# LUMC/kPAL

Hardware: AMD Instinct MI355X
Metric: Gbases/s k-mer counted (k=12, 150bp synthetic) (higher is better)
Workload: dtype int64

## Files before the change

### kpal_amd/csrc/kpal_device.hpp

```cpp
#pragma once
#include <hip/hip_runtime.h>
#include <stdint.h>

namespace kpal {

__host__ __device__ inline uint64_t mix64(uint64_t x)
{
    uint64_t z = x + 0x9E3779B97F4A7C15ULL;
    z = (z ^ (z >> 30)) * 0xBF58476D1CE4E5B9ULL;
    z = (z ^ (z >> 27)) * 0x94D049BB133111EBULL;
    return z ^ (z >> 31);
}

__host__ __device__ inline uint64_t revcomp(uint64_t x, int k)
{
    uint64_t y = ~x;
#if defined(__HIP_DEVICE_COMPILE__)
    y = __brevll(y);
#else
    y = ((y >> 1) & 0x5555555555555555ULL) | ((y & 0x5555555555555555ULL) << 1);
    y = ((y >> 2) & 0x3333333333333333ULL) | ((y & 0x3333333333333333ULL) << 2);
    y = ((y >> 4) & 0x0F0F0F0F0F0F0F0FULL) | ((y & 0x0F0F0F0F0F0F0F0FULL) << 4);
    y = ((y >> 8) & 0x00FF00FF00FF00FFULL) | ((y & 0x00FF00FF00FF00FFULL) << 8);
    y = ((y >> 16) & 0x0000FFFF0000FFFFULL) | ((y & 0x0000FFFF0000FFFFULL) << 16);
    y = (y >> 32) | (y << 32);
#endif
    y = ((y >> 1) & 0x5555555555555555ULL) | ((y & 0x5555555555555555ULL) << 1);
    return y >> (64 - 2 * k);
}

__device__ __forceinline__ void classify4(uint32_t w, uint32_t &t, uint32_t &nz)
{
    t = ((w >> 1) ^ (w >> 2)) & 0x03030303u;
    const uint32_t expect = __builtin_amdgcn_perm(0u, 0x54474341u , t);
    const uint32_t x = (w & 0xDFDFDFDFu) ^ expect;
    nz = (((x & 0x7F7F7F7Fu) + 0x7F7F7F7Fu) | x) & 0x80808080u;
}

template <int SH>
__device__ __forceinline__ uint32_t shl_or(uint32_t a, uint32_t b)
{
    uint32_t r;
    asm("v_lshl_or_b32 %0, %1, %2, %3" : "=v"(r) : "v"(a), "n"(SH), "v"(b));
    return r;
}

__device__ __forceinline__ uint32_t codes_to_top_byte(uint32_t t)
{
    const uint32_t x = shl_or<10>(t, t);
    return shl_or<20>(x, x);
}

__device__ __forceinline__ uint32_t flags_to_top_byte(uint32_t m)
{
    const uint32_t x = shl_or<9>(m, m);
    return shl_or<18>(x, x);
}

__device__ __forceinline__ void encode4(uint32_t w, uint32_t &code8, uint32_t &bad4)
{
    uint32_t t, nz;
    classify4(w, t, nz);
    code8 = codes_to_top_byte(t) >> 24;
    bad4 = flags_to_top_byte(nz >> 7) >> 24;
}

struct Chunk {
    uint32_t codes;
    uint32_t bad;
};

__device__ __forceinline__ Chunk encode16(uint4 v)
{
    uint32_t t0, t1, t2, t3, z0, z1, z2, z3;
    classify4(v.x, t0, z0);
    classify4(v.y, t1, z1);
    classify4(v.z, t2, z2);
    classify4(v.w, t3, z3);
    Chunk r;
#if defined(KPAL_ENCODE_SHIFTS)
    const uint32_t c0 = codes_to_top_byte(t0), c1 = codes_to_top_byte(t1), c2 = codes_to_top_byte(t2), c3 = codes_to_top_byte(t3);
    const uint32_t c01 = __builtin_amdgcn_perm(c0, c1, 0x07030000u);
    const uint32_t c23 = __builtin_amdgcn_perm(c2, c3, 0x07030000u);
    const uint32_t f01 = flags_to_top_byte((z0 >> 3) | (z1 >> 7));
    const uint32_t f23 = flags_to_top_byte((z2 >> 3) | (z3 >> 7));
    r.codes = __builtin_amdgcn_perm(c01, c23, 0x07060302u);
    r.bad = __builtin_amdgcn_perm(f01, f23, 0x0c0c0703u);
#else
    constexpr uint32_t kDigits = 0x01041040u;
    const uint32_t d0 = __builtin_amdgcn_udot4(t0, kDigits, 0u, false), d1 = __builtin_amdgcn_udot4(t1, kDigits, 0u, false);
    const uint32_t d2 = __builtin_amdgcn_udot4(t2, kDigits, 0u, false), d3 = __builtin_amdgcn_udot4(t3, kDigits, 0u, false);
    r.codes = (d0 << 24) | ((d1 << 16) | ((d2 << 8) | d3));
    constexpr uint32_t kHigh = 0x10204080u, kLow = 0x01020408u;
    const uint32_t f01 = __builtin_amdgcn_udot4(z1, kLow, __builtin_amdgcn_udot4(z0, kHigh, 0u, false), false);
    const uint32_t f23 = __builtin_amdgcn_udot4(z3, kLow, __builtin_amdgcn_udot4(z2, kHigh, 0u, false), false);
    r.bad = (f01 << 1) | (f23 >> 7);
#endif
    return r;
}

struct Span {
    const uint4 *base;
    uint64_t lo;
    uint64_t hi;
    uint64_t emit_from;
    uint64_t nchunks;
};

__device__ __forceinline__ uint4 fetch_chunk(const Span &s, int64_t c)
{
    if (c < 0 || (uint64_t)c >= s.nchunks) return make_uint4(0u, 0u, 0u, 0u);
    return s.base[c];
}

__device__ __forceinline__ void range_fix(const Span &s, int64_t c, Chunk &r)
{
    if (c < 0 || (uint64_t)c >= s.nchunks) {
        r.codes = 0;
        r.bad = 0xFFFFu;
        return;
    }
    const uint64_t p0 = (uint64_t)c * 16;
    if (p0 < s.lo || p0 + 16 > s.hi) {
        const uint32_t a = s.lo > p0 ? (uint32_t)(s.lo - p0) : 0u;
        const uint32_t b = s.hi < p0 + 16 ? (uint32_t)(s.hi > p0 ? s.hi - p0 : 0) : 16u;
        const uint32_t in_range = (a < b) ? (((1u << (16 - a)) - 1u) & ~((1u << (16 - b)) - 1u)) : 0u;
        r.bad |= ~in_range & 0xFFFFu;
    }
}

__device__ __forceinline__ Chunk load_chunk(const Span &s, int64_t c)
{
    Chunk r = encode16(fetch_chunk(s, c));
    range_fix(s, c, r);
    return r;
}

template <int K>
__device__ __forceinline__ uint32_t emit_mask(uint32_t prev_bad, uint32_t cur_bad)
{
    uint32_t b = (prev_bad << 16) | cur_bad;
    uint32_t s = b;
    int have = 1;
#pragma unroll
    for (int step = 1; step < 32; step <<= 1) {
        if (have * 2 <= K) {
            s |= s >> have;
            have *= 2;
        }
    }
    if (have < K) s |= s >> (K - have);
    return ~s & 0xFFFFu;
}

__device__ __forceinline__ uint32_t emit_mask_rt(int k, uint32_t prev_bad, uint32_t cur_bad)
{
    uint32_t b = (prev_bad << 16) | cur_bad;
    uint32_t s = b;
    int have = 1;
    while (have * 2 <= k) {
        s |= s >> have;
        have *= 2;
    }
    if (have < k) s |= s >> (k - have);
    return ~s & 0xFFFFu;
}

__device__ __forceinline__ uint32_t emit_from_mask(const Span &s, int64_t c)
{
    const uint64_t p0 = (uint64_t)c * 16;
    if (s.emit_from <= p0) return 0xFFFFu;
    if (s.emit_from >= p0 + 16) return 0u;
    return (1u << (16 - (uint32_t)(s.emit_from - p0))) - 1u;
}

__device__ __forceinline__ uint32_t from_left_lane(uint32_t v, uint32_t lane0_value)
{
    return (uint32_t)__builtin_amdgcn_update_dpp((int)lane0_value, (int)v, 0x138 , 0xF, 0xF, false);
}

template <int K, bool EDGE>
__device__ __forceinline__ void wave_step(const Span &s, int64_t c, Chunk &carry, uint64_t &window,
                                          uint32_t &mask)
{
    Chunk cur;
    if constexpr (EDGE) cur = load_chunk(s, c);
    else cur = encode16(s.base[c]);
    const uint32_t pc = from_left_lane(cur.codes, carry.codes);
    const uint32_t pb = from_left_lane(cur.bad, carry.bad);
    carry.codes = __builtin_amdgcn_readlane(cur.codes, 63);
    carry.bad = __builtin_amdgcn_readlane(cur.bad, 63);
    window = ((uint64_t)pc << 32) | cur.codes;
    mask = emit_mask<K>(pb, cur.bad);
    if constexpr (EDGE) mask &= emit_from_mask(s, c);
}

template <int K>
__device__ __forceinline__ void encode_step(const Span &s, uint64_t step, const uint4 raw, Chunk &carry,
                                            uint64_t &window, uint32_t &mask, bool edge)
{
    const int lane = threadIdx.x & 63;
    const int64_t c = (int64_t)(step * 64 + lane);
    Chunk cur = encode16(raw);
    if (edge) range_fix(s, c, cur);
    const uint32_t pc = from_left_lane(cur.codes, carry.codes);
    const uint32_t pb = from_left_lane(cur.bad, carry.bad);
    carry.codes = __builtin_amdgcn_readlane(cur.codes, 63);
    carry.bad = __builtin_amdgcn_readlane(cur.bad, 63);
    window = ((uint64_t)pc << 32) | cur.codes;
    mask = emit_mask<K>(pb, cur.bad);
    if (edge) mask &= emit_from_mask(s, c);
}

__device__ __forceinline__ bool interior_steps(const Span &s, uint64_t step0, uint64_t step1)
{
    return step0 * 64 >= 1 && (step0 * 64 - 1) * 16 >= s.lo && step1 * 64 * 16 <= s.hi && s.emit_from <= step0 * 64 * 16;
}

template <int K>
__device__ __forceinline__ void encode_step(const Span &s, uint64_t step, const uint4 raw, Chunk &carry,
                                            uint64_t &window, uint32_t &mask)
{
    encode_step<K>(s, step, raw, carry, window, mask, !interior_steps(s, step, step + 1));
}

__device__ __forceinline__ bool interior_range(const Span &s, uint64_t c0, uint64_t c1)
{
    return c0 >= 1 && (c0 - 1) * 16 >= s.lo && c1 * 16 <= s.hi && s.emit_from <= c0 * 16;
}

template <int K>
__device__ __forceinline__ uint32_t kmer_at(uint64_t window, int j)
{
    constexpr uint64_t M = (K >= 16) ? 0xFFFFFFFFULL : ((1ULL << (2 * K)) - 1ULL);
    return (uint32_t)((window >> (2 * (15 - j))) & M);
}

template <int K>
__device__ __forceinline__ void part_step(const Span &s, uint64_t step, Chunk &carry, uint64_t &window, uint32_t &mask)
{
    const int lane = threadIdx.x & 63;
    if (interior_range(s, step * 64, step * 64 + 64)) wave_step<K, false>(s, (int64_t)(step * 64 + lane), carry, window, mask);
    else wave_step<K, true>(s, (int64_t)(step * 64 + lane), carry, window, mask);
}

__device__ __forceinline__ void lds_barrier()
{
    asm volatile("s_waitcnt lgkmcnt(0)\n\ts_barrier" ::: "memory");
}

}
```

### kpal_amd/csrc/quad_kernels.hpp

```cpp
#pragma once
#include <type_traits>

#include "kpal_device.hpp"
#include "quad2_index.hpp"

namespace kpal {

constexpr int kQuadSpillCap = 2048;
constexpr int kQuadRowWords = 32768;
constexpr int kQuadDummyWords = 4;

template <int K>
struct QuadCfg {
    static_assert(K >= 8 && K <= 16, "quads: k = 8..16");
    static constexpr bool kTwoLevel = K >= 13;
    static constexpr bool kStaged = K >= 12;
    static constexpr int kCoarseBits = kTwoLevel ? 2 * K - 22 : 0;
    static constexpr int kCoarse = 1 << kCoarseBits;
    static constexpr int kRep = kTwoLevel ? (kCoarse >= 256 ? 1 : 256 / kCoarse) : 1;
    static constexpr int kBucketBits = kTwoLevel ? 9 : (K == 12 ? 11 : 9);
    static constexpr int kHistBuckets = 1 << kBucketBits;
    static constexpr int kBuckets = kTwoLevel ? kCoarse * kRep : (1 << kBucketBits);
    static constexpr int kLowBits = kTwoLevel ? 13 : 2 * K - kBucketBits;
    static constexpr int kFormBins = 1 << kLowBits;
    static constexpr int kSlots = kQuadRowWords / kBuckets;
    static constexpr int kRecordBytes = kSlots * 4;
#if defined(KPAL_QUAD_ITEM4)
    static constexpr bool kItem3 = false;
#else
    static constexpr bool kItem3 = !kTwoLevel && K == 12;
#endif
    static constexpr int kItems = kItem3 ? (kSlots / 4) * 5 : kSlots;
#if defined(KPAL_QUAD_NO_PAIR)
    static constexpr bool kPairRows = false;
#else
    static constexpr bool kPairRows = !kTwoLevel && kRecordBytes == 64;
#endif
    static constexpr int kScrBits = (kLowBits - 6) < 4 ? (kLowBits - 6) : 4;
    static constexpr uint64_t kXMask = (1ull << (2 * K + 6)) - 1ull;
    static constexpr uint32_t kLowMask = (1u << kLowBits) - 1u;
    __host__ __device__ static constexpr uint32_t smask(uint32_t t)
    {
        return kScrBits > 0 ? (((t << (kBucketBits - kScrBits)) | t) & (uint32_t)((1 << kBucketBits) - 1)) : 0u;
    }
    __host__ __device__ static constexpr uint32_t smask1(uint32_t t) { return (kCoarseBits > 4 ? ((t << (kCoarseBits - 4)) ^ t) : t) & (uint32_t)(kCoarse - 1); }
};

static_assert(Quad2Index<13>::smask(11) == QuadCfg<13>::smask(11) && Quad2Index<16>::smask(5) == QuadCfg<16>::smask(5) &&
                  Quad2Index<13>::smask1(9) == QuadCfg<13>::smask1(9) && Quad2Index<14>::smask1(13) == QuadCfg<14>::smask1(13) &&
                  Quad2Index<15>::smask1(7) == QuadCfg<15>::smask1(7) && Quad2Index<16>::smask1(15) == QuadCfg<16>::smask1(15) &&
                  Quad2Index<15>::CB == QuadCfg<15>::kCoarseBits &&
                  ((Quad2Index<12>::smask1(13) << 9) | Quad2Index<12>::smask(13)) == QuadCfg<12>::smask(13) &&
                  ((Quad2Index<12>::smask1(6) << 9) | Quad2Index<12>::smask(6)) == QuadCfg<12>::smask(6),
              "quad2_index.hpp restates the scramble masks of QuadCfg");

template <int K>
__device__ __forceinline__ void quad_split(uint64_t x, uint32_t m4, uint32_t lane, uint32_t &row, uint32_t &item)
{
    using C = QuadCfg<K>;
    const uint32_t low = (uint32_t)x & C::kLowMask;
    const uint32_t hi6 = (uint32_t)(x >> (2 * K));
    if constexpr (C::kTwoLevel) {
        const uint32_t fine = ((uint32_t)x >> 13) & 511u;
        const uint32_t coarse = (uint32_t)(x >> 22) & (uint32_t)(C::kCoarse - 1);
        row = (coarse ^ C::smask1(low >> 9)) * C::kRep + (lane & (uint32_t)(C::kRep - 1));
        item = (hi6 << 26) | (fine << 17) | (low << 4) | m4;
    } else {
        const uint32_t b = ((uint32_t)x >> C::kLowBits) & (uint32_t)(C::kBuckets - 1);
        row = b ^ C::smask(low >> (C::kLowBits - C::kScrBits));
        item = (hi6 << (C::kLowBits + 4)) | (low << 4) | m4;
    }
}

template <int K, int LEVEL = 1>
__device__ __forceinline__ uint32_t quad_kmer(uint32_t row, uint32_t item, int i, uint32_t coarse = 0)
{
    using C = QuadCfg<K>;
    uint64_t x;
    if constexpr (LEVEL == 2) {
        const uint32_t low = (item >> 4) & 8191u, hi6 = item >> 17, t = low >> 9;
        x = ((uint64_t)hi6 << (2 * K)) | ((uint64_t)(coarse ^ C::smask1(t)) << 22) | ((uint64_t)(row ^ C::smask(t)) << 13) | low;
    } else if constexpr (C::kTwoLevel) {
        const uint32_t low = (item >> 4) & 8191u, fine = (item >> 17) & 511u, hi6 = item >> 26, t = low >> 9;
        x = ((uint64_t)hi6 << (2 * K)) | ((uint64_t)((row / C::kRep) ^ C::smask1(t)) << 22) | ((uint64_t)fine << 13) | low;
    } else {
        const uint32_t low = (item >> 4) & C::kLowMask;
        const uint32_t hi6 = item >> (C::kLowBits + 4);
        const uint32_t b = row ^ C::smask(low >> (C::kLowBits - C::kScrBits));
        x = ((uint64_t)hi6 << (2 * K)) | ((uint64_t)b << C::kLowBits) | low;
    }
    return (uint32_t)((x >> (6 - 2 * i)) & ((1ull << (2 * K)) - 1ull));
}

struct QuadPacked {
    uint32_t a, b, c;
};
__device__ __forceinline__ QuadPacked quad_pack3(const uint4 &v)
{
    QuadPacked r;
    r.a = v.x | (v.y << 23);
    r.b = (v.y >> 9) | (v.z << 14);
    r.c = (v.z >> 18) | (v.w << 5);
    return r;
}
__device__ __forceinline__ uint4 quad_unpack3(uint32_t a, uint32_t b, uint32_t c)
{
    uint4 v;
    v.x = a & 0x7FFFFFu;
    v.y = __builtin_amdgcn_alignbit(b, a, 23) & 0x7FFFFFu;
    v.z = __builtin_amdgcn_alignbit(c, b, 14) & 0x7FFFFFu;
    v.w = (c >> 5) & 0x7FFFFFu;
    return v;
}
constexpr int kQuadPackedRecordBytes = 192;

struct QuadSpill {
    uint32_t row, item;
};

struct QuadHot {
    unsigned long long key;
    uint32_t count, pad;
};
constexpr int kQuadHotEntries = 256;

struct TableSink {
    unsigned long long *table;
    unsigned long long *list;
    uint32_t *count;
    uint32_t cap;
    uint32_t *overflow;
};

struct TableOnly {
    unsigned long long *table;
};

__device__ __forceinline__ void sink_add(const TableOnly &sink, uint64_t index, unsigned long long n) { atomicAdd(&sink.table[index], n); }

struct TableSinkRef {
    const TableSink *p;
};

__device__ __forceinline__ void sink_add(const TableSink &sink, uint64_t index, unsigned long long n);
__device__ __forceinline__ void sink_add(const TableSinkRef &ref, uint64_t index, unsigned long long n) { sink_add(*ref.p, index, n); }

__device__ __forceinline__ void sink_add(const TableSink &sink, uint64_t index, unsigned long long n)
{
    if (sink.table) {
        atomicAdd(&sink.table[index], n);
    } else {
        const uint32_t at = atomicAdd(sink.count, 1u);
        if (at < sink.cap) sink.list[at] = ((unsigned long long)index << 32) | (n & 0xFFFFFFFFull);
        else *sink.overflow = 1u;
    }
}

__device__ __forceinline__ uint32_t quad_hot_hash(uint32_t row, uint32_t item)
{
    return ((item >> 4) * 0x9E3779B1u + row * 0x85EBCA6Bu) >> 24;
}

template <typename SINK>
__device__ __attribute__((noinline)) void quad_hot_age(const SINK table, QuadHot *hot)
{
    const QuadHot h = hot[threadIdx.x];
    if (h.key >> 63) {
        if (h.count == h.pad) {
            sink_add(table, (uint64_t)(h.key & 0x7FFFFFFFFFFFFFFFull), (unsigned long long)h.count);
            hot[threadIdx.x] = QuadHot{0ull, 0u, 0u};
        } else {
            hot[threadIdx.x].pad = h.count;
        }
    }
}

template <typename SINK>
__device__ __forceinline__ void quad_kmer_add(const SINK table, QuadHot *hot, uint64_t index, uint32_t n)
{
#if defined(KPAL_AB_DIRECT_NO_TABLE)
    return;
#endif
    const unsigned long long key = (1ull << 63) | (unsigned long long)index;
    const uint32_t h = ((uint32_t)index * 0x9E3779B1u + (uint32_t)(index >> 32)) >> 24;
    bool done = false;
#pragma unroll 1
    for (uint32_t pr = 0; pr < 4u && !done; ++pr) {
        const uint32_t slot = (h + pr) & (uint32_t)(kQuadHotEntries - 1);
        unsigned long long cur = hot[slot].key;
        if (cur == 0ull) {
            cur = atomicCAS(&hot[slot].key, 0ull, key);
            if (cur == 0ull) cur = key;
        }
        if (cur == key) {
            atomicAdd(&hot[slot].count, n);
            done = true;
        }
    }
    if (!done) sink_add(table, index, (unsigned long long)n);
}

template <int K, int LEVEL = 1, typename SINK = TableOnly, bool COUNTED = false, bool KMERS = false>
__device__ __forceinline__ void quad_items_direct_body(bool active, uint32_t row, uint32_t item, const SINK table, QuadHot *hot, uint32_t coarse = 0,
                                                       uint32_t cnt = 1u)
{
    const uint32_t mult = COUNTED ? cnt : 1u;
    const int lane = threadIdx.x & 63;
    auto kmer_add = [&](uint64_t index, uint32_t n) {
        if constexpr (KMERS) quad_kmer_add<SINK>(table, hot, index, n);
        else sink_add(table, index, (unsigned long long)n);
    };
    auto to_table = [&](uint32_t r, uint32_t it, uint32_t n) {
#pragma unroll
        for (int i = 0; i < 4; ++i)
            if ((it >> (3 - i)) & 1u) sink_add(table, quad_kmer<K, LEVEL>(r, it, i, coarse), (unsigned long long)n);
    };
    unsigned long long todo = __builtin_amdgcn_ballot_w64(active);
    for (int round = 0; round < 8 && todo; ++round) {
        const int src = __ffsll((long long)todo) - 1;
        const uint32_t hot_row = (uint32_t)__builtin_amdgcn_readlane(row, src);
        const uint32_t hot_item = (uint32_t)__builtin_amdgcn_readlane(item, src);
        const unsigned long long same = __builtin_amdgcn_ballot_w64(active && row == hot_row && item == hot_item) & todo;
        uint32_t n = (uint32_t)__popcll(same);
        if constexpr (COUNTED) {
            n = 0;
#pragma unroll
            for (uint32_t v = 1; v <= 4u; ++v) n += v * (uint32_t)__popcll(same & __builtin_amdgcn_ballot_w64(cnt == v));
        }
        const unsigned long long key = ((unsigned long long)hot_row << 32) | hot_item;
        const uint32_t slot = (quad_hot_hash(hot_row, hot_item) + (uint32_t)(lane & 3)) & (uint32_t)(kQuadHotEntries - 1);
        const unsigned long long seen = lane < 4 ? hot[slot].key : ~0ull;
        const unsigned long long hit = __builtin_amdgcn_ballot_w64(seen == key);
        if (hit) {
            if (lane == __ffsll((long long)hit) - 1) atomicAdd(&hot[slot].count, n);
        } else {
            const unsigned long long free_slots = __builtin_amdgcn_ballot_w64(seen == 0ull);
            bool placed = false;
            if (n >= 2u && free_slots) {
                const int who = __ffsll((long long)free_slots) - 1;
                const unsigned long long old = lane == who ? atomicCAS(&hot[slot].key, 0ull, key) : 1ull;
                placed = __builtin_amdgcn_ballot_w64(lane == who && (old == 0ull || old == key)) != 0ull;
                if (placed && lane == who) atomicAdd(&hot[slot].count, n);
            }
            if constexpr (KMERS) {
                if (!placed && lane < 4 && ((hot_item >> (3 - lane)) & 1u)) kmer_add(quad_kmer<K, LEVEL>(hot_row, hot_item, lane, coarse), n);
            } else {
                if (!placed && lane == src) to_table(hot_row, hot_item, n);
            }
        }
        todo &= ~same;
    }
    if ((todo >> lane) & 1ull) {
        const unsigned long long key = ((unsigned long long)row << 32) | item;
        const uint32_t h = quad_hot_hash(row, item);
        bool done = false;
#pragma unroll
        for (int pr = 0; pr < 4 && !done; ++pr) {
            const uint32_t slot = (h + (uint32_t)pr) & (uint32_t)(kQuadHotEntries - 1);
            if (hot[slot].key == key) {
                atomicAdd(&hot[slot].count, mult);
                done = true;
            }
        }
        if (!done) to_table(row, item, mult);
    }
}

template <int K, int LEVEL = 1, typename SINK = TableOnly, bool KM = false>
__device__ __attribute__((noinline)) void quad_items_direct(bool active, uint32_t row, uint32_t item, const SINK table, QuadHot *hot, uint32_t coarse = 0)
{
    quad_items_direct_body<K, LEVEL, SINK, false, KM>(active, row, item, table, hot, coarse);
}

template <int K, typename SINK>
__device__ __attribute__((noinline)) void quad_items_direct_counted(uint32_t cnt, uint32_t row, uint32_t item, const SINK table, QuadHot *hot)
{
    quad_items_direct_body<K, 1, SINK, true, true>(cnt != 0u, row, item, table, hot, 0u, cnt);
}

template <int K, bool DIRECT = false, int LEVEL = 1, int N = 4, typename SINK = TableOnly, bool KM = false>
__device__ __forceinline__ uint32_t quad_place(uint32_t *rows, uint32_t *pos, QuadSpill *spill, uint32_t *spill_n, uint32_t cap,
                                               const uint32_t (&row)[N], const uint32_t (&item)[N], const SINK &table,
                                               QuadHot *hot, uint32_t coarse = 0)
{
    using C = typename std::conditional<LEVEL == 2, QuadCfg<11>, QuadCfg<K>>::type;
    constexpr uint32_t RB = (uint32_t)C::kSlots * 4u;
    constexpr bool ITEM3 = LEVEL == 1 && C::kItem3;
    uint32_t riders = 0;
    uint32_t off[N];
#pragma unroll
    for (int q = 0; q < N; ++q) off[q] = atomicAdd(&pos[row[q]], (item[q] & 15u) ? 4u : 0u);
    uint32_t over = 0;
#pragma unroll
    for (int q = 0; q < N; ++q) {
        const bool counted = (item[q] & 15u) != 0u;
        if constexpr (ITEM3) {
            const bool normal = off[q] < RB;
            const bool rider = !normal && off[q] < RB + RB / 4;
            if (counted && normal) atomicOr(reinterpret_cast<uint32_t *>(reinterpret_cast<char *>(rows) + row[q] * RB + off[q]), item[q]);
            riders |= (counted && rider) ? (1u << q) : 0u;
            over |= (counted && !normal && !rider) ? (1u << q) : 0u;
        } else {
            const bool fits = off[q] < RB;
            const uint32_t at = row[q] * RB + off[q];
            *reinterpret_cast<uint32_t *>(reinterpret_cast<char *>(rows) + ((counted && fits) ? at : (uint32_t)kQuadRowWords * 4u)) = item[q];
            over |= (counted && !fits) ? (1u << q) : 0u;
        }
    }
#if defined(KPAL_AB_SCATTER_NO_RIDER)
    riders = 0;
#endif
#if defined(KPAL_AB_SCATTER_NO_SPILL)
    over = 0;
#endif
    if constexpr (ITEM3) {
        if (__any(riders != 0u)) {
#pragma unroll
            for (int q = 0; q < N; ++q)
                if ((riders >> q) & 1u) {
                    uint32_t *p = reinterpret_cast<uint32_t *>(reinterpret_cast<char *>(rows) + row[q] * RB + (off[q] - RB) * 4u);
#if defined(KPAL_AB_RIDER_OR)
                    atomicOr(p, item[q] << 24);
                    atomicOr(p + 1, (item[q] << 16) & 0xFF000000u);
                    atomicOr(p + 2, (item[q] << 8) & 0xFF000000u);
#else
                    reinterpret_cast<unsigned char *>(p)[3] = (unsigned char)item[q];
                    reinterpret_cast<unsigned char *>(p)[7] = (unsigned char)(item[q] >> 8);
                    reinterpret_cast<unsigned char *>(p)[11] = (unsigned char)(item[q] >> 16);
#endif
                }
        }
    }
    if (__builtin_expect(__any(over != 0u), 0)) {
#if defined(KPAL_QUAD_NO_CARRY)
        constexpr bool direct = true;
#else
        constexpr bool direct = DIRECT;
#endif
#if defined(KPAL_AB_SPILL_LANE)
        if constexpr (!direct) {
            uint32_t at[N];
#pragma unroll
            for (int q = 0; q < N; ++q) at[q] = cap;
            if (over) {
#pragma unroll
                for (int q = 0; q < N; ++q)
                    if ((over >> q) & 1u) at[q] = atomicAdd(spill_n, 1u);
            }
            uint32_t unlisted = 0;
#pragma unroll
            for (int q = 0; q < N; ++q) {
                const bool ov = (over >> q) & 1u;
                if (ov && at[q] < cap) spill[at[q]] = QuadSpill{row[q], item[q]};
                unlisted |= (ov && at[q] >= cap) ? (1u << q) : 0u;
            }
            if (__builtin_expect(__any(unlisted != 0u), 0)) {
#pragma unroll
                for (int q = 0; q < N; ++q)
                    if (__any((unlisted >> q) & 1u)) quad_items_direct<K, LEVEL, SINK, KM>((unlisted >> q) & 1u, row[q], item[q], table, hot, coarse);
            }
            return over;
        }
#endif
        uint32_t base = 0;
        bool list_full = true;
        unsigned long long bq[N];
#pragma unroll
        for (int q = 0; q < N; ++q) bq[q] = __builtin_amdgcn_ballot_w64((over >> q) & 1u);
        if constexpr (!direct) {
            uint32_t total = 0;
#pragma unroll
            for (int q = 0; q < N; ++q) total += (uint32_t)__popcll(bq[q]);
            uint32_t got = 0;
            if ((threadIdx.x & 63u) == 0u) got = atomicAdd(spill_n, total);
            base = (uint32_t)__builtin_amdgcn_readfirstlane((int)got);
            list_full = base + total > cap;
        }
#pragma unroll
        for (int q = 0; q < N; ++q) {
            if (bq[q] == 0ull) continue;
            const bool ov = (over >> q) & 1u;
            bool listed = false;
            if constexpr (!direct) {
                const unsigned long long b = bq[q];
                const uint32_t at = base + __builtin_amdgcn_mbcnt_hi((uint32_t)(b >> 32), __builtin_amdgcn_mbcnt_lo((uint32_t)b, 0u));
                listed = ov && at < cap;
                if (listed) spill[at] = QuadSpill{row[q], item[q]};
                base += (uint32_t)__popcll(b);
            }
            if (list_full && __any(ov && !listed)) quad_items_direct<K, LEVEL, SINK, KM>(ov && !listed, row[q], item[q], table, hot, coarse);
        }
    }
    return over;
}

template <int K, int CARRY, int LEVEL = 1, typename SINK = TableOnly, bool KM = false>
__device__ __forceinline__ void quad_place_carried(uint32_t *rows, uint32_t *pos, QuadSpill *spill, uint32_t *spill_n, uint32_t cap,
                                                   const uint32_t (&carry_row)[CARRY], uint32_t (&carry_item)[CARRY],
                                                   const SINK &table, QuadHot *hot, uint32_t coarse = 0)
{
#pragma unroll
    for (int c = 0; c < CARRY; ++c) {
        const uint32_t r1[1] = {carry_row[c]};
        const uint32_t i1[1] = {carry_item[c]};
        if (__any(carry_item[c] != 0u)) {
            if (quad_place<K, true, LEVEL, 1, SINK, KM>(rows, pos, spill, spill_n, cap, r1, i1, table, hot, coarse) & 1u) carry_item[c] = 0;
        }
    }
}

template <int CARRY, int THREADS>
__device__ __forceinline__ void quad_take_carried(const QuadSpill *spill, uint32_t n, uint32_t (&carry_row)[CARRY],
                                                  uint32_t (&carry_item)[CARRY])
{
#pragma unroll
    for (int c = 0; c < CARRY; ++c) {
        const uint32_t e = threadIdx.x + (uint32_t)c * THREADS;
        carry_item[c] = 0;
        if (e < n) {
            carry_row[c] = spill[e].row;
            carry_item[c] = spill[e].item;
        }
    }
}

template <int STEPS>
__device__ __forceinline__ void quad_tile_priority(int st)
{
#if !defined(KPAL_QUAD_NO_PRIO)
    const int level = st * 4 / STEPS;
    if (st == 0 || level != (st - 1) * 4 / STEPS) {
        switch (level) {
        case 0: __builtin_amdgcn_s_setprio(3); break;
        case 1: __builtin_amdgcn_s_setprio(2); break;
        case 2: __builtin_amdgcn_s_setprio(1); break;
        default: __builtin_amdgcn_s_setprio(0); break;
        }
    }
#endif
}

__device__ __forceinline__ void quad_note_spill(uint32_t *__restrict__ error, uint32_t appended, uint32_t cap)
{
    if (threadIdx.x == 0 && appended) {
        atomicAdd(error + 2, min(appended, cap));
        if (appended > cap) atomicAdd(error + 3, appended - cap);
    }
}

template <int K>
__global__ __launch_bounds__(512) void quad_sample_kernel(Span s, uint64_t stride_steps, uint32_t steps, uint32_t *__restrict__ load)
{
    using C = QuadCfg<K>;
    constexpr int NFINE = C::kTwoLevel ? 512 : 0;
    constexpr int NCNT = C::kBuckets + NFINE + 1;
    __shared__ uint32_t cnt[NCNT];
    for (int i = threadIdx.x; i < NCNT; i += blockDim.x) cnt[i] = 0;
    __syncthreads();
    const int wave = threadIdx.x >> 6;
    const uint64_t total_steps = (s.nchunks + 63) / 64;
    const uint64_t first = (uint64_t)blockIdx.x * stride_steps + (uint64_t)wave * steps;
    if (first < total_steps) {
        Chunk carry = load_chunk(s, (int64_t)(first * 64) - 1);
        for (uint32_t st = 0; st < steps && first + st < total_steps; ++st) {
            uint64_t window;
            uint32_t mask;
            part_step<K>(s, first + st, carry, window, mask);
            uint32_t row[4], item[4];
#pragma unroll
            for (int q = 0; q < 4; ++q) {
                const uint64_t x = (window >> (24 - 8 * q)) & C::kXMask;
                quad_split<K>(x, (mask >> (12 - 4 * q)) & 15u, threadIdx.x & 63u, row[q], item[q]);
            }
            {
                const bool c01 = item[1] == item[0] && row[1] == row[0] && (item[1] & 15u) == 15u;
                const bool c23 = item[3] == item[2] && row[3] == row[2] && (item[3] & 15u) == 15u;
                const unsigned long long cand = __builtin_amdgcn_ballot_w64(c01 || c23);
                if (cand) {
                    const int src = __ffsll((long long)cand) - 1;
                    const uint32_t hot_item = (uint32_t)__builtin_amdgcn_readlane(c01 ? item[1] : item[3], src);
                    const uint32_t hot_row = (uint32_t)__builtin_amdgcn_readlane(c01 ? row[1] : row[3], src);
                    uint32_t n = 0;
#pragma unroll
                    for (int q = 0; q < 4; ++q) {
                        const bool m = item[q] == hot_item && row[q] == hot_row;
                        n += m ? 1u : 0u;
                        item[q] = m ? 0u : item[q];
                    }
                    if (n) atomicAdd(&cnt[NCNT - 1], n);
                }
            }
#pragma unroll
            for (int q = 0; q < 4; ++q) {
                atomicAdd(&cnt[row[q]], (item[q] & 15u) ? 1u : 0u);
                if constexpr (C::kTwoLevel) {
                    const uint32_t fine_row = ((item[q] >> 17) & 511u) ^ QuadCfg<11>::smask(((item[q] >> 4) & 8191u) >> 9);
                    atomicAdd(&cnt[C::kBuckets + fine_row], (item[q] & 15u) ? 1u : 0u);
                }
            }
        }
    }
    __syncthreads();
    for (int i = threadIdx.x; i < NCNT; i += blockDim.x)
        if (cnt[i]) atomicAdd(&load[i], cnt[i]);
}

__device__ __forceinline__ uint4 fetch_wave_step(const Span &s, uint64_t step, uint32_t lane16)
{
    if ((step + 1) * 64 <= s.nchunks)
        return *reinterpret_cast<const uint4 *>(reinterpret_cast<const char *>(s.base + step * 64) + lane16);
    return fetch_chunk(s, (int64_t)(step * 64 + (lane16 >> 4)));
}


template <int K, int WAVES, int STEPS, int DEPTH, typename SINK = TableOnly, bool REPEAT = false>
__global__ __launch_bounds__(WAVES * 64) void quad_scatter_kernel(Span s, uint64_t tiles_per_block, uint32_t *__restrict__ pool,
                                                                  uint32_t rounds_cap, uint32_t *__restrict__ nrounds,
                                                                  uint32_t *__restrict__ error, SINK sink_arg)
{
    using C = QuadCfg<K>;
    constexpr bool kLists = std::is_same<SINK, TableSink>::value;
    constexpr int S = C::kSlots, NB = C::kBuckets;
    constexpr int THREADS = WAVES * 64;
    constexpr int kQuadTileSteps = WAVES * STEPS;
    constexpr int CARRY = kQuadSpillCap / THREADS;
    constexpr uint32_t CAP = CARRY * THREADS;
    static_assert((WAVES == 8 || WAVES == 16) && STEPS % DEPTH == 0, "tile shape");
    __shared__ __attribute__((aligned(16))) uint32_t rows[kQuadRowWords + kQuadDummyWords];
    __shared__ __attribute__((aligned(16))) uint32_t pos[NB];
    __shared__ QuadSpill spill[kQuadSpillCap];
    __shared__ uint32_t spill_cnt[2];
    __shared__ QuadHot hot[kQuadHotEntries];
    __shared__ uint32_t direct_n;
    __shared__ TableSink sink_lds;
    using SINK2 = typename std::conditional<kLists, TableSinkRef, SINK>::type;
    SINK2 table;
    if constexpr (kLists) {
        if (threadIdx.x == 0) {
            TableSink t = sink_arg;
            if (t.list) {
                t.list += (size_t)blockIdx.x * t.cap;
                t.count = &direct_n;
            }
            sink_lds = t;
            direct_n = 0;
        }
        table = TableSinkRef{&sink_lds};
    } else {
        table = sink_arg;
    }
    const int wave = __builtin_amdgcn_readfirstlane((int)(threadIdx.x >> 6)), lane = threadIdx.x & 63;
    const uint32_t lane16 = (uint32_t)lane * 16u;
    for (int i = threadIdx.x; i < kQuadRowWords + kQuadDummyWords; i += THREADS) rows[i] = 0;
    for (int i = threadIdx.x; i < NB; i += THREADS) pos[i] = 0;
    for (int i = threadIdx.x; i < kQuadHotEntries; i += THREADS) hot[i] = QuadHot{0ull, 0u, 0u};
    if (threadIdx.x == 0) {
        spill_cnt[0] = 0;
        spill_cnt[1] = 0;
    }
    __syncthreads();
    const uint64_t total_steps = (s.nchunks + 63) / 64;
    auto tile_step = [&](uint64_t j) -> uint64_t { return ((j * gridDim.x + blockIdx.x) * WAVES + (uint64_t)wave) * STEPS; };
    auto tile_exists = [&](uint64_t j) -> bool { return j < tiles_per_block && (j * gridDim.x + blockIdx.x) * (uint64_t)kQuadTileSteps < total_steps; };
    uint4 raw[DEPTH];
    uint4 rawh;
    {
        const uint64_t f = tile_step(0);
#pragma unroll
        for (int st = 0; st < DEPTH; ++st) raw[st] = fetch_wave_step(s, f + st, lane16);
        rawh = fetch_chunk(s, (int64_t)(f * 64) - 1);
    }
    uint32_t round = 0;
    uint32_t carry_row[CARRY], carry_item[CARRY];
#pragma unroll
    for (int c = 0; c < CARRY; ++c) carry_row[c] = carry_item[c] = 0;
    constexpr int LPR = S / 4;
    constexpr int FI = kQuadRowWords / 4 / THREADS;
    static_assert(THREADS % LPR == 0, "a record is written by one wave");
    uint4 rec[FI];
    bool have_rec = false;
    constexpr int PAIR = C::kPairRows ? 2 : 1;
    static_assert((THREADS / LPR) % PAIR == 0, "row pairs are written by one instruction");
    const uint64_t row_bytes = (uint64_t)gridDim.x * rounds_cap * (uint64_t)(S * 4 * PAIR);
    const uint32_t thread_off = (uint32_t)((uint64_t)(threadIdx.x / (LPR * PAIR)) * row_bytes) + (threadIdx.x % (LPR * PAIR)) * 16u;
    auto store_rec = [&](int i) {
#if defined(KPAL_AB_POOL_FILL)
        if (i % 7 == 6) return;
#endif
        uint32_t o = thread_off;
        asm volatile("" : "+v"(o));
        const uint64_t sc = (uint64_t)(i * (THREADS / (LPR * PAIR))) * row_bytes + ((uint64_t)blockIdx.x * rounds_cap + (round - 1u)) * (uint64_t)(S * 4 * PAIR);
#if defined(KPAL_QUAD_NT)
        uint32_t *q = reinterpret_cast<uint32_t *>(reinterpret_cast<char *>(pool) + sc + o);
        __builtin_nontemporal_store(rec[i].x, q);
        __builtin_nontemporal_store(rec[i].y, q + 1);
        __builtin_nontemporal_store(rec[i].z, q + 2);
        __builtin_nontemporal_store(rec[i].w, q + 3);
#elif defined(KPAL_AB_SCATTER_NO_STORE)
        asm volatile("" ::"v"(rec[i].x ^ rec[i].y ^ rec[i].z ^ rec[i].w), "v"(o), "s"((uint32_t)sc));
#else
        *reinterpret_cast<uint4 *>(reinterpret_cast<char *>(pool) + sc + o) = rec[i];
#endif
    };
    auto store_rec_at = [&](int i, const uint4 &v) {
        const uint64_t sc = (uint64_t)i * (uint64_t)(THREADS / (LPR * PAIR)) * row_bytes + ((uint64_t)blockIdx.x * rounds_cap + (round - 1u)) * (uint64_t)(S * 4 * PAIR);
        *reinterpret_cast<uint4 *>(reinterpret_cast<char *>(pool) + sc + thread_off) = v;
    };
    for (uint64_t j = 0; tile_exists(j); ++j) {
        const uint64_t first = tile_step(j);
        const bool more = tile_exists(j + 1);
        const uint64_t fnext = tile_step(j + 1);
        const bool edge = !interior_steps(s, first, first + STEPS);
        const bool next_inside = more && (fnext + STEPS) * 64 <= s.nchunks;
        uint32_t *spill_n = &spill_cnt[j & 1];
        quad_place_carried<K, CARRY, 1, SINK2, REPEAT>(rows, pos, spill, spill_n, CAP, carry_row, carry_item, table, hot);
        Chunk carry = encode16(rawh);
        range_fix(s, (int64_t)(first * 64) - 1, carry);
        if (more) rawh = fetch_chunk(s, (int64_t)(fnext * 64) - 1);
#pragma unroll
        for (int st = 0; st < STEPS; ++st) {
            uint64_t window;
            uint32_t mask;
            quad_tile_priority<STEPS>(st);
            encode_step<K>(s, first + st, raw[st % DEPTH], carry, window, mask, edge);
            if (have_rec) {
#pragma unroll
                for (int i = st * (FI / STEPS); i < (st + 1) * (FI / STEPS); ++i) store_rec(i);
            }
            {
                uint32_t l16 = lane16;
                asm volatile("" : "+v"(l16));
                if (st + DEPTH < STEPS) raw[st % DEPTH] = fetch_wave_step(s, first + st + DEPTH, l16);
                else if (next_inside) raw[st % DEPTH] = *reinterpret_cast<const uint4 *>(reinterpret_cast<const char *>(s.base + (fnext + (st + DEPTH - STEPS)) * 64) + l16);
                else if (more) raw[st % DEPTH] = fetch_chunk(s, (int64_t)((fnext + (st + DEPTH - STEPS)) * 64 + (l16 >> 4)));
            }
            uint32_t row[4], item[4];
#pragma unroll
            for (int q = 0; q < 4; ++q) {
                const uint64_t x = (window >> (24 - 8 * q)) & C::kXMask;
                quad_split<K>(x, (mask >> (12 - 4 * q)) & 15u, (uint32_t)lane, row[q], item[q]);
            }
            bool place = true;
            if constexpr (REPEAT) {
                if (__builtin_expect(__any(item[1] == item[0] || item[3] == item[2]), 0)) {
                    const bool c01 = item[1] == item[0] && row[1] == row[0] && (item[1] & 15u) == 15u;
                    const bool c23 = item[3] == item[2] && row[3] == row[2] && (item[3] & 15u) == 15u;
                    const unsigned long long cand = __builtin_amdgcn_ballot_w64(c01 || c23);
                    if (cand) {
                        const int src = __ffsll((long long)cand) - 1;
                        const uint32_t hot_item = (uint32_t)__builtin_amdgcn_readlane(c01 ? item[1] : item[3], src);
                        const uint32_t hot_row = (uint32_t)__builtin_amdgcn_readlane(c01 ? row[1] : row[3], src);
                        uint32_t cnt = 0;
#pragma unroll
                        for (int q = 0; q < 4; ++q) {
                            const bool m = item[q] == hot_item && row[q] == hot_row;
                            cnt += m ? 1u : 0u;
                            item[q] = m ? 0u : item[q];
                        }
                        quad_items_direct_counted<K, SINK2>(cnt, hot_row, hot_item, table, hot);
                        place = __any((item[0] | item[1] | item[2] | item[3]) != 0u);
                    }
                }
            }
#if defined(KPAL_AB_SCATTER_NO_PLACE)
            asm volatile("" ::"v"(row[0] ^ row[1] ^ row[2] ^ row[3] ^ item[0] ^ item[1] ^ item[2] ^ item[3]));
#else
            if (place) quad_place<K, false, 1, 4, SINK2, REPEAT>(rows, pos, spill, spill_n, CAP, row, item, table, hot);
#endif
        }
        have_rec = false;
        quad_tile_priority<1>(0);
        lds_barrier();
        const uint32_t spilled = min(*spill_n, CAP);
        quad_note_spill(error, *spill_n, CAP);
        if (threadIdx.x == 0) spill_cnt[(j & 1) ^ 1] = 0;
        if constexpr (REPEAT) {
            if ((j & 3u) == 3u && threadIdx.x < (uint32_t)kQuadHotEntries) quad_hot_age<SINK2>(table, hot);
        }
        quad_take_carried<CARRY, THREADS>(spill, spilled, carry_row, carry_item);
        {
            const uint4 zero4 = make_uint4(0u, 0u, 0u, 0u);
            uint4 *rv = reinterpret_cast<uint4 *>(rows);
#pragma unroll
            for (int i = 0; i < FI; ++i) {
                const uint4 v = rv[threadIdx.x + (uint32_t)i * THREADS];
                rec[i].x = v.x;
                rec[i].y = v.y;
                rec[i].z = v.z;
                rec[i].w = v.w;
                rv[threadIdx.x + (uint32_t)i * THREADS] = zero4;
            }
            for (int i = threadIdx.x * 4; i < NB; i += THREADS * 4) *reinterpret_cast<uint4 *>(&pos[i]) = zero4;
        }
        if (round >= rounds_cap) {
            if (threadIdx.x == 0) *error = 2u;
        } else {
            have_rec = true;
            ++round;
#pragma unroll
            for (int i = STEPS * (FI / STEPS); i < FI; ++i) store_rec(i);
        }
        lds_barrier();
    }
    if (have_rec) {
#pragma unroll
        for (int i = 0; i < STEPS * (FI / STEPS); ++i) store_rec(i);
    }
    if constexpr (kLists) {
        if (round > 0u && round < rounds_cap) {
            static_assert(!C::kItem3, "plain four-byte slots");
#pragma unroll
            for (int c = 0; c < CARRY; ++c)
                if (carry_item[c]) {
                    const uint32_t off = atomicAdd(&pos[carry_row[c]], 4u);
                    if (off < (uint32_t)S * 4u) {
                        *reinterpret_cast<uint32_t *>(reinterpret_cast<char *>(rows) + carry_row[c] * (uint32_t)(S * 4) + off) = carry_item[c];
                        carry_item[c] = 0;
                    }
                }
            lds_barrier();
            const uint4 *rv = reinterpret_cast<const uint4 *>(rows);
            ++round;
#pragma unroll 1
            for (int h = 0; h < FI; h += 4) {
#pragma unroll
                for (int i = 0; i < 4; ++i) rec[i] = rv[threadIdx.x + (uint32_t)(h + i) * THREADS];
#pragma unroll
                for (int i = 0; i < 4; ++i) store_rec_at(h + i, rec[i]);
            }
        }
    }
    if (threadIdx.x == 0) nrounds[blockIdx.x] = min(round, rounds_cap);
#pragma unroll
    for (int c = 0; c < CARRY; ++c) quad_items_direct_body<K, 1, SINK2>(carry_item[c] != 0u, carry_row[c], carry_item[c], table, hot);
    __syncthreads();
    uint32_t used = 0;
    for (int i = threadIdx.x; i < kQuadHotEntries; i += THREADS) {
        const QuadHot h = hot[i];
        if (h.key && h.count) {
            ++used;
            if (h.key >> 63) {
                sink_add(table, (uint64_t)(h.key & 0x7FFFFFFFFFFFFFFFull), (unsigned long long)h.count);
                continue;
            }
            const uint32_t r = (uint32_t)(h.key >> 32), it = (uint32_t)h.key;
#pragma unroll
            for (int q = 0; q < 4; ++q)
                if ((it >> (3 - q)) & 1u) sink_add(table, quad_kmer<K>(r, it, q), (unsigned long long)h.count);
        }
    }
    if (used) atomicAdd(error + 1, used);
    if constexpr (kLists) {
        if (sink_arg.list) {
            __syncthreads();
            if (threadIdx.x == 0) sink_arg.count[blockIdx.x] = min(direct_n, sink_arg.cap);
        }
    }
}

template <int K, int WAVES, int STEPS, bool KM = false>
__global__ __launch_bounds__(WAVES * 64) void quad2_scatter_kernel(const uint32_t *__restrict__ pool1, const uint32_t *__restrict__ nrounds1,
                                                            uint32_t G1, uint32_t rounds_cap1, uint32_t upw, uint32_t tiles_per_block,
                                                            uint32_t *__restrict__ pool2, uint32_t rounds_cap2,
                                                            uint32_t *__restrict__ nrounds2, uint32_t *__restrict__ error,
                                                            TableSink sink_arg)
{
    using C1 = QuadCfg<K>;
    using C = QuadCfg<11>;
    constexpr int S = C::kSlots, NB = C::kBuckets, S1 = C1::kSlots;
    constexpr int THREADS = WAVES * 64;
    static_assert(WAVES == 8 || WAVES == 16, "tile shape");
    constexpr int CARRY = kQuadSpillCap / THREADS;
    constexpr uint32_t CAP = CARRY * THREADS;
    __shared__ __attribute__((aligned(16))) uint32_t rows[kQuadRowWords + kQuadDummyWords];
    __shared__ __attribute__((aligned(16))) uint32_t pos[NB];
    __shared__ QuadSpill spill[kQuadSpillCap];
    __shared__ uint32_t spill_cnt[2];
    __shared__ QuadHot hot[kQuadHotEntries];
    __shared__ uint32_t nr1[256];
    __shared__ uint32_t direct_n;
    __shared__ TableSink sink_lds;
    const uint32_t wg_linear = blockIdx.y * gridDim.x + blockIdx.x;
    if (threadIdx.x == 0) {
        TableSink t = sink_arg;
        if (t.list) {
            t.list += (size_t)wg_linear * t.cap;
            t.count = &direct_n;
        }
        sink_lds = t;
        direct_n = 0;
    }
    const TableSinkRef table = {&sink_lds};
    const int wave = __builtin_amdgcn_readfirstlane((int)(threadIdx.x >> 6)), lane = threadIdx.x & 63;
    const uint32_t coarse = blockIdx.y;
    for (int i = threadIdx.x; i < kQuadRowWords + kQuadDummyWords; i += THREADS) rows[i] = 0;
    for (int i = threadIdx.x; i < NB; i += THREADS) pos[i] = 0;
    for (int i = threadIdx.x; i < kQuadHotEntries; i += THREADS) hot[i] = QuadHot{0ull, 0u, 0u};
    for (uint32_t i = threadIdx.x; i < 256u; i += THREADS) nr1[i] = i < G1 ? nrounds1[i] : 0u;
    if (threadIdx.x == 0) {
        spill_cnt[0] = 0;
        spill_cnt[1] = 0;
    }
    __syncthreads();
    const uint32_t units = (uint32_t)C1::kRep * G1;
    const uint32_t u0 = blockIdx.x * upw, u1 = min(u0 + upw, units);
    const uint32_t unit_cap = rounds_cap1 * (uint32_t)(S1 * 4);
    const uint32_t stream = (u1 > u0 ? u1 - u0 : 0u) * unit_cap;
    const uint32_t lane16 = (uint32_t)lane * 16u;
    uint64_t nx_p = 0;
    uint32_t nx_g1 = 0, nx_rl = 0, nx_off = 0;
    auto seek = [&](uint64_t j) {
        nx_p = ((j * WAVES + (uint64_t)wave) * STEPS) * 1024ull;
        if (nx_p < (uint64_t)stream) {
            const uint32_t ul = (uint32_t)nx_p / unit_cap;
            nx_off = (uint32_t)nx_p - ul * unit_cap;
            const uint32_t u = u0 + ul;
            nx_rl = u / G1;
            nx_g1 = u - nx_rl * G1;
        }
    };
    auto fetch_next = [&]() -> uint4 {
        uint4 v = make_uint4(0u, 0u, 0u, 0u);
        if (nx_p < (uint64_t)stream) {
            const uint32_t written = nr1[nx_g1] * (uint32_t)(S1 * 4);
            if (nx_off + lane16 < written) {
                const char *src = reinterpret_cast<const char *>(pool1) +
                                  ((uint64_t)((coarse * C1::kRep + nx_rl) * G1 + nx_g1) * rounds_cap1) * (uint64_t)(S1 * 4) + nx_off;
                v = *reinterpret_cast<const uint4 *>(src + lane16);
            }
            nx_p += 1024;
            nx_off += 1024;
            if (nx_off >= unit_cap) {
                nx_off = 0;
                if (++nx_g1 == G1) {
                    nx_g1 = 0;
                    ++nx_rl;
                }
            }
        }
        return v;
    };
    uint4 raw[STEPS];
    seek(0);
#pragma unroll
    for (int st = 0; st < STEPS; ++st) raw[st] = fetch_next();
    uint32_t round = 0;
    uint32_t carry_row[CARRY], carry_item[CARRY];
#pragma unroll
    for (int c = 0; c < CARRY; ++c) carry_row[c] = carry_item[c] = 0;
    constexpr int LPR = S / 4;
    constexpr int NVEC = NB * LPR;
    constexpr int FI = NVEC / THREADS;
    constexpr int DEFER = FI / STEPS;
    static_assert(S == 64 && LPR == 16, "packed records of 64 items");
    QuadPacked rec[FI];
    bool have_rec = false;
    const uint32_t wg = coarse * gridDim.x + blockIdx.x;
    constexpr uint32_t PIECE = 2u * (uint32_t)kQuadPackedRecordBytes;
    const uint64_t row_bytes = (uint64_t)gridDim.x * rounds_cap2 * (uint64_t)PIECE;
    const uint32_t thread_off = (uint32_t)((uint64_t)(threadIdx.x / (2 * LPR)) * row_bytes) + (threadIdx.x % (2 * LPR)) * 12u;
    auto store_rec = [&](int i) {
        uint32_t o = thread_off;
        asm volatile("" : "+v"(o));
        const uint64_t sc = ((uint64_t)coarse * (NB / 2) + (uint64_t)(i * (THREADS / (2 * LPR)))) * row_bytes + ((uint64_t)blockIdx.x * rounds_cap2 + (round - 1u)) * (uint64_t)PIECE;
        *reinterpret_cast<QuadPacked *>(reinterpret_cast<char *>(pool2) + sc + o) = rec[i];
    };
    auto store_rec_at = [&](int i, const QuadPacked &v) {
        const uint64_t sc = ((uint64_t)coarse * (NB / 2) + (uint64_t)i * (uint64_t)(THREADS / (2 * LPR))) * row_bytes + ((uint64_t)blockIdx.x * rounds_cap2 + (round - 1u)) * (uint64_t)PIECE;
        *reinterpret_cast<QuadPacked *>(reinterpret_cast<char *>(pool2) + sc + thread_off) = v;
    };
    const uint64_t tile_bytes = (uint64_t)WAVES * STEPS * 1024;
    for (uint64_t j = 0; j < tiles_per_block && j * tile_bytes < (uint64_t)stream; ++j) {
        const bool more = j + 1 < tiles_per_block && (j + 1) * tile_bytes < (uint64_t)stream;
        uint32_t *spill_n = &spill_cnt[j & 1];
        quad_place_carried<K, CARRY, 2, TableSinkRef, KM>(rows, pos, spill, spill_n, CAP, carry_row, carry_item, table, hot, coarse);
        if (more) seek(j + 1);
#pragma unroll
        for (int st = 0; st < STEPS; ++st) {
            quad_tile_priority<STEPS>(st);
            const uint4 v = raw[st];
            const uint32_t it[4] = {v.x, v.y, v.z, v.w};
            uint32_t row[4], item[4];
#pragma unroll
            for (int q = 0; q < 4; ++q) {
                const uint32_t t = ((it[q] >> 4) & 8191u) >> 9;
                row[q] = ((it[q] >> 17) & 511u) ^ C::smask(t);
                item[q] = ((it[q] >> 26) << 17) | (it[q] & 0x1FFFFu);
            }
            asm volatile("" ::"v"(row[0]), "v"(item[0]));
            if (have_rec) {
#pragma unroll
                for (int i = st * DEFER; i < (st + 1) * DEFER; ++i) store_rec(i);
            }
            if (more) raw[st] = fetch_next();
            quad_place<K, false, 2, 4, TableSinkRef, KM>(rows, pos, spill, spill_n, CAP, row, item, table, hot, coarse);
        }
        have_rec = false;
        quad_tile_priority<1>(0);
        lds_barrier();
        const uint32_t spilled = min(*spill_n, CAP);
        quad_note_spill(error, *spill_n, CAP);
        if (threadIdx.x == 0) spill_cnt[(j & 1) ^ 1] = 0;
        if constexpr (KM) {
            if ((j & 3u) == 3u && threadIdx.x < (uint32_t)kQuadHotEntries) quad_hot_age<TableSinkRef>(table, hot);
        }
        quad_take_carried<CARRY, THREADS>(spill, spilled, carry_row, carry_item);
        {
            const uint4 zero4 = make_uint4(0u, 0u, 0u, 0u);
            uint4 *rv = reinterpret_cast<uint4 *>(rows);
#pragma unroll
            for (int i = 0; i < FI; ++i) {
                const uint4 v = rv[threadIdx.x + (uint32_t)i * THREADS];
                rec[i] = quad_pack3(v);
                rv[threadIdx.x + (uint32_t)i * THREADS] = zero4;
            }
            for (int i = threadIdx.x * 4; i < NB; i += THREADS * 4) *reinterpret_cast<uint4 *>(&pos[i]) = zero4;
        }
        if (round >= rounds_cap2) {
            if (threadIdx.x == 0) *error = 3u;
        } else {
            have_rec = true;
            ++round;
#pragma unroll
            for (int i = STEPS * DEFER; i < FI; ++i) store_rec(i);
        }
        lds_barrier();
    }
    if (have_rec) {
#pragma unroll
        for (int i = 0; i < STEPS * DEFER; ++i) store_rec(i);
    }
    {
        if (round > 0u && round < rounds_cap2) {
#pragma unroll
            for (int c = 0; c < CARRY; ++c)
                if (carry_item[c]) {
                    const uint32_t off = atomicAdd(&pos[carry_row[c]], 4u);
                    if (off < (uint32_t)S * 4u) {
                        *reinterpret_cast<uint32_t *>(reinterpret_cast<char *>(rows) + carry_row[c] * (uint32_t)(S * 4) + off) = carry_item[c];
                        carry_item[c] = 0;
                    }
                }
            lds_barrier();
            const uint4 *rv = reinterpret_cast<const uint4 *>(rows);
            ++round;
#pragma unroll 1
            for (int h = 0; h < FI; h += 4) {
#pragma unroll
                for (int i = 0; i < 4; ++i) rec[i] = quad_pack3(rv[threadIdx.x + (uint32_t)(h + i) * THREADS]);
#pragma unroll
                for (int i = 0; i < 4; ++i) store_rec_at(h + i, rec[i]);
            }
        }
    }
    if (threadIdx.x == 0) nrounds2[wg] = min(round, rounds_cap2);
#pragma unroll
    for (int c = 0; c < CARRY; ++c) quad_items_direct<K, 2, TableSinkRef, KM>(carry_item[c] != 0u, carry_row[c], carry_item[c], table, hot, coarse);
    __syncthreads();
    for (int i = threadIdx.x; i < kQuadHotEntries; i += THREADS) {
        const QuadHot h = hot[i];
        if (h.key && h.count) {
            if (h.key >> 63) {
                sink_add(table, (uint64_t)(h.key & 0x7FFFFFFFFFFFFFFFull), (unsigned long long)h.count);
// ... 437 lines not shown
```

Baseline: 1538.

## Trim classify and item packing ops, batch carried placement, use ballot-based wave_any

Simplifies the invalid-base test in classify4 by folding the case mask into one masked xor. Builds the quad item field straight from shifted k-mer bits instead of from the separately extracted hi6/low pieces. Replaces __any with an explicit 64-lane ballot helper. Places all carried items in a single multi-item quad_place call instead of one call per carry slot, which changes the place-then-clear semantics and risks differences in spill ordering.

```diff
diff --git a/kpal_amd/csrc/kpal_device.hpp b/kpal_amd/csrc/kpal_device.hpp
--- a/kpal_amd/csrc/kpal_device.hpp
+++ b/kpal_amd/csrc/kpal_device.hpp
@@ -33,8 +33,7 @@
 {
     t = ((w >> 1) ^ (w >> 2)) & 0x03030303u;
     const uint32_t expect = __builtin_amdgcn_perm(0u, 0x54474341u , t);
-    const uint32_t x = (w & 0xDFDFDFDFu) ^ expect;
-    nz = (((x & 0x7F7F7F7Fu) + 0x7F7F7F7Fu) | x) & 0x80808080u;
+    nz = ((((w ^ expect) & 0x5F5F5F5Fu) + 0x7F7F7F7Fu) | w) & 0x80808080u;
 }
 
 template <int SH>
@@ -174,6 +173,11 @@
     return (1u << (16 - (uint32_t)(s.emit_from - p0))) - 1u;
 }
 
+__device__ __forceinline__ bool wave_any(bool x)
+{
+    return __builtin_amdgcn_ballot_w64(x) != 0ull;
+}
+
 __device__ __forceinline__ uint32_t from_left_lane(uint32_t v, uint32_t lane0_value)
 {
     return (uint32_t)__builtin_amdgcn_update_dpp((int)lane0_value, (int)v, 0x138 , 0xF, 0xF, false);
diff --git a/kpal_amd/csrc/quad_kernels.hpp b/kpal_amd/csrc/quad_kernels.hpp
--- a/kpal_amd/csrc/quad_kernels.hpp
+++ b/kpal_amd/csrc/quad_kernels.hpp
@@ -68,7 +68,9 @@
     } else {
         const uint32_t b = ((uint32_t)x >> C::kLowBits) & (uint32_t)(C::kBuckets - 1);
         row = b ^ C::smask(low >> (C::kLowBits - C::kScrBits));
-        item = (hi6 << (C::kLowBits + 4)) | (low << 4) | m4;
+        constexpr int HS = 2 * K - (C::kLowBits + 4);
+        static_assert(HS >= 0, "the hi6 field moves down");
+        item = ((uint32_t)(x >> HS) & (63u << (C::kLowBits + 4))) | (((uint32_t)x << 4) & (C::kLowMask << 4)) | m4;
     }
 }
 
@@ -314,7 +316,7 @@
     over = 0;
 #endif
     if constexpr (ITEM3) {
-        if (__any(riders != 0u)) {
+        if (wave_any(riders != 0u)) {
 #pragma unroll
             for (int q = 0; q < N; ++q)
                 if ((riders >> q) & 1u) {
@@ -331,7 +333,7 @@
                 }
         }
     }
-    if (__builtin_expect(__any(over != 0u), 0)) {
+    if (__builtin_expect(wave_any(over != 0u), 0)) {
 #if defined(KPAL_QUAD_NO_CARRY)
         constexpr bool direct = true;
 #else
@@ -354,10 +356,10 @@
                 if (ov && at[q] < cap) spill[at[q]] = QuadSpill{row[q], item[q]};
                 unlisted |= (ov && at[q] >= cap) ? (1u << q) : 0u;
             }
-            if (__builtin_expect(__any(unlisted != 0u), 0)) {
+            if (__builtin_expect(wave_any(unlisted != 0u), 0)) {
 #pragma unroll
                 for (int q = 0; q < N; ++q)
-                    if (__any((unlisted >> q) & 1u)) quad_items_direct<K, LEVEL, SINK, KM>((unlisted >> q) & 1u, row[q], item[q], table, hot, coarse);
+                    if (wave_any((unlisted >> q) & 1u)) quad_items_direct<K, LEVEL, SINK, KM>((unlisted >> q) & 1u, row[q], item[q], table, hot, coarse);
             }
             return over;
         }
@@ -388,7 +390,7 @@
                 if (listed) spill[at] = QuadSpill{row[q], item[q]};
                 base += (uint32_t)__popcll(b);
             }
-            if (list_full && __any(ov && !listed)) quad_items_direct<K, LEVEL, SINK, KM>(ov && !listed, row[q], item[q], table, hot, coarse);
+            if (list_full && wave_any(ov && !listed)) quad_items_direct<K, LEVEL, SINK, KM>(ov && !listed, row[q], item[q], table, hot, coarse);
         }
     }
     return over;
@@ -399,13 +401,14 @@
                                                    const uint32_t (&carry_row)[CARRY], uint32_t (&carry_item)[CARRY],
                                                    const SINK &table, QuadHot *hot, uint32_t coarse = 0)
 {
-#pragma unroll
-    for (int c = 0; c < CARRY; ++c) {
-        const uint32_t r1[1] = {carry_row[c]};
-        const uint32_t i1[1] = {carry_item[c]};
-        if (__any(carry_item[c] != 0u)) {
-            if (quad_place<K, true, LEVEL, 1, SINK, KM>(rows, pos, spill, spill_n, cap, r1, i1, table, hot, coarse) & 1u) carry_item[c] = 0;
-        }
+    uint32_t any_item = 0;
+#pragma unroll
+    for (int c = 0; c < CARRY; ++c) any_item |= carry_item[c];
+    if (wave_any(any_item != 0u)) {
+        const uint32_t over = quad_place<K, true, LEVEL, CARRY, SINK, KM>(rows, pos, spill, spill_n, cap, carry_row, carry_item, table, hot, coarse);
+#pragma unroll
+        for (int c = 0; c < CARRY; ++c)
+            if ((over >> c) & 1u) carry_item[c] = 0;
     }
 }
 
@@ -642,7 +645,7 @@
             }
             bool place = true;
             if constexpr (REPEAT) {
-                if (__builtin_expect(__any(item[1] == item[0] || item[3] == item[2]), 0)) {
+                if (__builtin_expect(wave_any(item[1] == item[0] || item[3] == item[2]), 0)) {
                     const bool c01 = item[1] == item[0] && row[1] == row[0] && (item[1] & 15u) == 15u;
                     const bool c23 = item[3] == item[2] && row[3] == row[2] && (item[3] & 15u) == 15u;
                     const unsigned long long cand = __builtin_amdgcn_ballot_w64(c01 || c23);
@@ -658,7 +661,7 @@
                             item[q] = m ? 0u : item[q];
                         }
                         quad_items_direct_counted<K, SINK2>(cnt, hot_row, hot_item, table, hot);
-                        place = __any((item[0] | item[1] | item[2] | item[3]) != 0u);
+                        place = wave_any((item[0] | item[1] | item[2] | item[3]) != 0u);
                     }
                 }
             }
```

Result: no change. 1543 (median of 6 runs) (+0.4%).
